# Natasha-R/Flood-Prediction-GAN

Measured on AMD Instinct MI355X. Metric: GAN training images/sec (512x512, PairedAttention), higher is better.
Workload: dtype f32

## Files before the change

### flood-prediction-gan_amd/csrc/conv_common.hpp

```cpp
#pragma once
#include "fg_common.hpp"

typedef _Float16 f16x8 __attribute__((ext_vector_type(8)));
typedef _Float16 f16x4 __attribute__((ext_vector_type(4)));
typedef _Float16 f16x2 __attribute__((ext_vector_type(2)));
typedef float f32x2 __attribute__((ext_vector_type(2)));

namespace fgc {

struct ConvBatch {
    fg_conv_problem p[4];
    int count;
    int ntiles_n[4];
    int blk_start[5];
    int interleave;
};

__device__ __forceinline__ int div_small(int n, int d) {
    int q = (int)((float)n * __builtin_amdgcn_rcpf((float)d));
    const int r = n - q * d;
    q += r >= d ? 1 : (r < 0 ? -1 : 0);
    return q;
}

// ... 13 lines not shown

__device__ __forceinline__ float pow2_of(float m) {
    if (!(m > 0.f) || !(m < 3.0e38f)) return 1.f;
    int e;
    frexpf(m, &e);
    return ldexpf(1.f, 14 - e);
}

__device__ __forceinline__ float pow2_scale_max(const float* amax) {
    unsigned b = __float_as_uint(amax[threadIdx.x & (FG_AMAX_SHARDS - 1)]) & 0x7fffffffu;
#pragma unroll
    for (int off = 1; off < FG_AMAX_SHARDS; off <<= 1) b = max(b, (unsigned)__shfl_xor((int)b, off));
    return __uint_as_float(b);
}

__device__ __forceinline__ float pow2_scale(const float* amax) {
    unsigned b = amax ? __float_as_uint(amax[threadIdx.x & (FG_AMAX_SHARDS - 1)]) & 0x7fffffffu : 0u;
#pragma unroll
    for (int off = 1; off < FG_AMAX_SHARDS; off <<= 1) b = max(b, (unsigned)__shfl_xor((int)b, off));
    return pow2_of(__uint_as_float(b));
}

__device__ __forceinline__ void split_f16(const float (&v)[8], float s, f16x8& h, f16x8& l) {
#pragma unroll
    for (int e = 0; e < 4; ++e) {
        const f32x2 x = f32x2{v[2 * e], v[2 * e + 1]} * s;
        const f16x2 hh = __builtin_convertvector(x, f16x2);
        const f16x2 ll = __builtin_convertvector(x - __builtin_convertvector(hh, f32x2), f16x2);
        h[2 * e] = hh[0];
        h[2 * e + 1] = hh[1];
        l[2 * e] = ll[0];
        l[2 * e + 1] = ll[1];
    }
}

__device__ __forceinline__ void split_pair_mix(float x0, float x1, float s, unsigned& h, unsigned& l) {
    unsigned hv, lv;
    asm("v_fma_mixlo_f16 %0, %1, %2, 0\n\t"
        "v_fma_mixhi_f16 %0, %3, %2, 0"
        : "=&v"(hv) : "v"(x0), "v"(s), "v"(x1));
    asm("v_fma_mixlo_f16 %0, %1, %2, -%4 op_sel_hi:[0,0,1]\n\t"
        "v_fma_mixhi_f16 %0, %3, %2, -%4 op_sel:[0,0,1] op_sel_hi:[0,0,1]"
        : "=&v"(lv) : "v"(x0), "v"(s), "v"(x1), "v"(hv));
    h = hv;
    l = lv;
}

template <int C>
__device__ __forceinline__ int swz_pixel(int x) {
    if constexpr (C == 64) return (x & 7) << 1;
    else return ((x >> 1) & 3) << 1;
}

int launch_fwd_f3(const ConvBatch& b, int nprob, int max_n, hipStream_t stream, int* rc);
bool f3_stats_ok(const fg_conv_problem* probs, int nprob, int max_n);

int launch_wgrad_f3(const fg_wgrad_problem& p, hipStream_t stream, int* rc);

int stem_wgrad_rows(const fg_wgrad_problem& p);
int launch_wgrad_stem(const fg_wgrad_problem& p, hipStream_t stream, int* rc);
int stem_fwd_rows(const fg_conv_problem& p);
int launch_fwd_stem(const fg_conv_problem& p, hipStream_t stream, int* rc);

}
```

### flood-prediction-gan_amd/csrc/conv_f3.hip

```cpp
#include <algorithm>

#include "conv_common.hpp"

namespace {

using fgc::ConvBatch;

__device__ __forceinline__ int swz_a(int row) { return ((row >> 1) & 1) ^ (((row >> 3) & 1) << 2); }
__device__ __forceinline__ int swz_b(int row) { return ((row >> 3) & 1) << 1; }

typedef __attribute__((address_space(3))) void lds_void;
typedef unsigned u32x4 __attribute__((ext_vector_type(4)));

__device__ __forceinline__ void split_scalar(const float (&v)[8], float s, f16x8& h, f16x8& l) {
#pragma unroll
    for (int e = 0; e < 4; ++e) {
        const float x0 = v[2 * e] * s, x1 = v[2 * e + 1] * s;
        const f16x2 hh = __builtin_convertvector(f32x2{x0, x1}, f16x2);
        const float r0 = x0 - (float)hh[0], r1 = x1 - (float)hh[1];
        const f16x2 ll = __builtin_convertvector(f32x2{r0, r1}, f16x2);
        h[2 * e] = hh[0];
        h[2 * e + 1] = hh[1];
        l[2 * e] = ll[0];
        l[2 * e + 1] = ll[1];
    }
}

template <int A_GL, int B_GL, int A_BYTES>
__device__ __forceinline__ void dma_stage(char* sb, int wave, __amdgpu_buffer_rsrc_t xr, __amdgpu_buffer_rsrc_t wr,
                                          const int* a_off, const int* b_off, int soff_a, int soff_b) {
#pragma unroll
    for (int i = 0; i < A_GL; ++i)
        __builtin_amdgcn_raw_ptr_buffer_load_lds(xr, (lds_void*)(sb + (wave * A_GL + i) * 1024), 16, a_off[i], soff_a,
                                                 0, 0);
#pragma unroll
    for (int i = 0; i < B_GL; ++i)
        __builtin_amdgcn_raw_ptr_buffer_load_lds(wr, (lds_void*)(sb + A_BYTES + (wave * B_GL + i) * 1024), 16, b_off[i],
                                                 soff_b, 0, 0);
}

__device__ __forceinline__ f32x4 mma_t(f16x8 a, f16x8 b, f32x4 c) {
    return __builtin_amdgcn_mfma_f32_16x16x32_f16(b, a, c, 0, 0, 0);
}

__device__ __forceinline__ int quad_yoff(const fg_conv_problem& P, int q) {
    const int y0 = (int)P.q_yoff[0], y1 = (int)P.q_yoff[1], y2 = (int)P.q_yoff[2], y3 = (int)P.q_yoff[3];
    return q == 0 ? y0 : q == 1 ? y1 : q == 2 ? y2 : y3;
}

constexpr int kYRecords = 0x7fffff00, kYOOB = 0x7ffffff0;

__device__ __forceinline__ void dma_piece(char* dst, __amdgpu_buffer_rsrc_t r, int voff, int soff) {
    __builtin_amdgcn_raw_ptr_buffer_load_lds(r, (lds_void*)dst, 16, voff, soff, 0, 0);
}

constexpr int cap63(int n) { return n < 63 ? n : 63; }

template <int N>
__device__ __forceinline__ void wait_vmcnt() {
    static_assert(N >= 0 && N <= 63, "vmcnt immediate (6 bits)");
    asm volatile("s_waitcnt vmcnt(%0)" ::"n"(N) : "memory");
}

__device__ __forceinline__ void wait_vmcnt_rt(int n) {
    switch (n < 63 ? n : 63) {
        case 0: wait_vmcnt<0>(); break;
        case 1: wait_vmcnt<1>(); break;
        case 2: wait_vmcnt<2>(); break;
        case 3: wait_vmcnt<3>(); break;
        case 4: wait_vmcnt<4>(); break;
        case 5: wait_vmcnt<5>(); break;
        case 6: wait_vmcnt<6>(); break;
        case 7: wait_vmcnt<7>(); break;
        case 8: wait_vmcnt<8>(); break;
        case 9: wait_vmcnt<9>(); break;
        case 10: wait_vmcnt<10>(); break;
        case 11: wait_vmcnt<11>(); break;
        case 12: wait_vmcnt<12>(); break;
        case 13: wait_vmcnt<13>(); break;
        case 14: wait_vmcnt<14>(); break;
        case 15: wait_vmcnt<15>(); break;
        case 16: wait_vmcnt<16>(); break;
        case 17: wait_vmcnt<17>(); break;
        case 18: wait_vmcnt<18>(); break;
        case 19: wait_vmcnt<19>(); break;
        case 20: wait_vmcnt<20>(); break;
        case 21: wait_vmcnt<21>(); break;
        case 22: wait_vmcnt<22>(); break;
        case 23: wait_vmcnt<23>(); break;
        case 24: wait_vmcnt<24>(); break;
        case 25: wait_vmcnt<25>(); break;
        case 26: wait_vmcnt<26>(); break;
        case 27: wait_vmcnt<27>(); break;
        case 28: wait_vmcnt<28>(); break;
        case 29: wait_vmcnt<29>(); break;
        case 30: wait_vmcnt<30>(); break;
        case 31: wait_vmcnt<31>(); break;
        case 32: wait_vmcnt<32>(); break;
        case 33: wait_vmcnt<33>(); break;
        case 34: wait_vmcnt<34>(); break;
        case 35: wait_vmcnt<35>(); break;
        case 36: wait_vmcnt<36>(); break;
        case 37: wait_vmcnt<37>(); break;
        case 38: wait_vmcnt<38>(); break;
        case 39: wait_vmcnt<39>(); break;
        case 40: wait_vmcnt<40>(); break;
        case 41: wait_vmcnt<41>(); break;
        case 42: wait_vmcnt<42>(); break;
        case 43: wait_vmcnt<43>(); break;
        case 44: wait_vmcnt<44>(); break;
        case 45: wait_vmcnt<45>(); break;
        case 46: wait_vmcnt<46>(); break;
        case 47: wait_vmcnt<47>(); break;
        case 48: wait_vmcnt<48>(); break;
        case 49: wait_vmcnt<49>(); break;
// ... 785 lines not shown
```

### flood-prediction-gan_amd/csrc/conv_wgrad_f3.hip

```cpp
#include "conv_common.hpp"

namespace {

typedef short s16x4 __attribute__((ext_vector_type(4)));
typedef __attribute__((address_space(3))) s16x4 lds_s16x4;

constexpr int BR = 32;
constexpr int TK = 256;

__device__ __forceinline__ int swz_tr(int row) { return ((row & 3) | (((row >> 3) & 1) << 2)) << 1; }

template <int COLS>
__device__ __forceinline__ int img_off(int row, int col) {
    return row * (COLS * 2) + (((col >> 3) ^ (swz_tr(row) & (COLS / 8 - 1))) << 4) + ((col & 7) << 1);
}

__device__ __forceinline__ f16x8 tr_frag(const char* base, int a0, int a1) {
    const s16x4 lo = __builtin_amdgcn_ds_read_tr16_b64_v4i16((lds_s16x4*)(base + a0));
    const s16x4 hi = __builtin_amdgcn_ds_read_tr16_b64_v4i16((lds_s16x4*)(base + a1));
    typedef short s16x8 __attribute__((ext_vector_type(8)));
    const s16x8 v = {lo[0], lo[1], lo[2], lo[3], hi[0], hi[1], hi[2], hi[3]};
    return __builtin_bit_cast(f16x8, v);
}

__device__ __forceinline__ void split4(const f32x4& v, float s, f16x4& h, f16x4& l) {
    typedef unsigned u32x2 __attribute__((ext_vector_type(2)));
    u32x2 hu, lu;
#pragma unroll
    for (int e = 0; e < 2; ++e) {
        unsigned a, b;
        fgc::split_pair_mix(v[2 * e], v[2 * e + 1], s, a, b);
        hu[e] = a;
        lu[e] = b;
    }
    h = __builtin_bit_cast(f16x4, hu);
    l = __builtin_bit_cast(f16x4, lu);
}

template <int TA, int SCH, int PS = 0>
__global__ void __launch_bounds__(512, 1)
conv_wgrad_f3_kernel(const fg_wgrad_problem P, int tiles_a, int tiles_k) {
    constexpr int NT = 512, NWA = TA / 64, NWK = 8 / NWA, WK = TK / NWK, TM = 4, TN = WK / 16;
    constexpr int SPT = BR * TK / 4 / NT;
    constexpr int IMGP = BR * TA * 2, IMGX = BR * TK * 2;
    constexpr int PL = IMGP + 64, XH = 2 * IMGP + 128, XL = XH + IMGX + 64;
    constexpr int BUF = XL + IMGX + 64;
    constexpr int kOOB = 0x7fffffff;
    __shared__ __attribute__((aligned(1024))) char smem[2 * BUF];

    const int tid = threadIdx.x, lane = tid & 63, wave = __builtin_amdgcn_readfirstlane(tid >> 6);
    const int wa = wave / NWK, wk = wave - (wave / NWK) * NWK;
    const int wid = fg::xcd_remap(blockIdx.x, gridDim.x);
    const int ntile = tiles_a * tiles_k;
    const int split = wid / ntile;
    const int tile = wid - split * ntile;
    const int ta = tile / tiles_k, tk = tile - (tile / tiles_k) * tiles_k;
    const int a0 = ta * TA, k0 = tk * TK;
    const int mab = P.m_a * P.m_b;
    const int M = P.m_img * mab;
    const int mbeg = split * P.m_chunk;
    const int mend = min(M, mbeg + P.m_chunk);
    const int K = P.kh * P.j_valid;
    const int nst = mend > mbeg ? (mend - mbeg + BR - 1) / BR : 0;

    const __amdgpu_buffer_rsrc_t pr = __builtin_amdgcn_make_buffer_rsrc((void*)P.p, 0, 0x7fffffff, 0x00020000);
    const __amdgpu_buffer_rsrc_t xr = __builtin_amdgcn_make_buffer_rsrc((void*)P.x, 0, 0x7fffffff, 0x00020000);
    const float sp = fgc::pow2_scale(P.p_absmax);
    const float sx = fgc::pow2_scale(P.x_absmax);

    const int col = (tid & 63) * 4;
    const int prow0 = wave;
    const bool p_slot = col < TA;
    const bool p_col_ok = p_slot && a0 + col < P.n_a;
    int x_koff = -1;
    {
        const int k = k0 + col;
        if (k < K) {
            const int r = k / P.j_valid;
            x_koff = r * (int)P.sxr + (k - r * P.j_valid);
        }
    }
    const int i32 = BR / mab, a32 = (BR - i32 * mab) / P.m_b, b32 = BR - i32 * mab - a32 * P.m_b;
    int wm[SPT], wi[SPT], wa_[SPT], wb[SPT];
#pragma unroll
    for (int i = 0; i < SPT; ++i) {
        wm[i] = mbeg + prow0 + 8 * i;
        fgc::decomp(min(wm[i], M - 1), P.m_b, mab, wi[i], wa_[i], wb[i]);
    }
    f32x4 rp[SPT], rx[SPT];
    auto load_slot = [&](int i) {
        {
            const bool ok = wm[i] < mend;
            const int pb = wi[i] * (int)P.spn + wa_[i] * (int)P.spa + wb[i] * (int)P.spb + a0 + col;
            const int xb = wi[i] * (int)P.sxn + wa_[i] * (int)P.sxa + wb[i] * (int)P.sxb + x_koff;
            rp[i] = __builtin_bit_cast(f32x4, __builtin_amdgcn_raw_buffer_load_b128(pr, ok && p_col_ok ? pb * 4 : kOOB, 0, 0));
            rx[i] = __builtin_bit_cast(f32x4, __builtin_amdgcn_raw_buffer_load_b128(xr, ok && x_koff >= 0 ? xb * 4 : kOOB, 0, 0));
            wm[i] += BR;
            wb[i] += b32;
            const int cb = wb[i] >= P.m_b;
            wb[i] -= cb ? P.m_b : 0;
            wa_[i] += a32 + cb;
            const int ca = wa_[i] >= P.m_a;
            wa_[i] -= ca ? P.m_a : 0;
            wi[i] += i32 + ca;
        }
    };
    auto load = [&]() {
#pragma unroll
        for (int i = 0; i < SPT; ++i) load_slot(i);
    };
    auto store_slot = [&](int buf, int i) {
        char* b = smem + buf * BUF;
        {
            f16x4 h, l;
            if (p_slot) {
                if constexpr (PS & 1) {
                    const int op = img_off<TA>(prow0 + 8 * i, col & ~7) + ((col & 4) ? PL : 0);
                    *reinterpret_cast<f16x8*>(b + op) = __builtin_bit_cast(f16x8, rp[i]);
                } else {
                    const int op = img_off<TA>(prow0 + 8 * i, col);
                    split4(rp[i], sp, h, l);
                    *reinterpret_cast<f16x4*>(b + op) = h;
                    *reinterpret_cast<f16x4*>(b + PL + op) = l;
                }
            }
            if constexpr (PS & 2) {
                const int ox = img_off<TK>(prow0 + 8 * i, col & ~7) + ((col & 4) ? XL : XH);
                *reinterpret_cast<f16x8*>(b + ox) = __builtin_bit_cast(f16x8, rx[i]);
            } else {
                const int ox = img_off<TK>(prow0 + 8 * i, col);
                split4(rx[i], sx, h, l);
                *reinterpret_cast<f16x4*>(b + XH + ox) = h;
                *reinterpret_cast<f16x4*>(b + XL + ox) = l;
            }
        }
    };
    auto store = [&](int buf) {
#pragma unroll
        for (int i = 0; i < SPT; ++i) store_slot(buf, i);
    };

    f32x4 acc[TM][TN];
#pragma unroll
    for (int tm = 0; tm < TM; ++tm)
#pragma unroll
        for (int tn = 0; tn < TN; ++tn) acc[tm][tn] = f32x4{0.f, 0.f, 0.f, 0.f};

    const int g = lane >> 4, q = (lane >> 2) & 3, p4 = (lane & 3) * 4;
    constexpr int TG = SCH == 0 ? (TN < 4 ? TN : 4) : TN / SPT;
    static_assert(TN % TG == 0 && (SCH == 0 || TN / TG == SPT), "groups");
    auto compute = [&](int buf, bool stage_next) {
        const char* b = smem + buf * BUF;
        f16x8 ah[TM], al[TM];
#pragma unroll
        for (int tm = 0; tm < TM; ++tm) {
            const int c = wa * 64 + tm * 16 + p4;
            const int o0 = img_off<TA>(8 * g + q, c), o1 = img_off<TA>(8 * g + 4 + q, c);
            ah[tm] = tr_frag(b, o0, o1);
            al[tm] = tr_frag(b + PL, o0, o1);
        }
#pragma unroll
        for (int t0 = 0; t0 < TN; t0 += TG) {
            f16x8 bh[TG], bl[TG];
#pragma unroll
            for (int t = 0; t < TG; ++t) {
                const int c = wk * WK + (t0 + t) * 16 + p4;
                const int o0 = img_off<TK>(8 * g + q, c), o1 = img_off<TK>(8 * g + 4 + q, c);
                bh[t] = tr_frag(b + XH, o0, o1);
                bl[t] = tr_frag(b + XL, o0, o1);
            }
            if constexpr (SCH == 1) {
                if (stage_next) store_slot(buf ^ 1, t0 / TG);
                load_slot(t0 / TG);
            }
#pragma unroll
            for (int tm = 0; tm < TM; ++tm)
#pragma unroll
                for (int t = 0; t < TG; ++t)
                    acc[tm][t0 + t] = __builtin_amdgcn_mfma_f32_16x16x32_f16(bh[t], al[tm], acc[tm][t0 + t], 0, 0, 0);
#pragma unroll
            for (int tm = 0; tm < TM; ++tm)
#pragma unroll
                for (int t = 0; t < TG; ++t)
                    acc[tm][t0 + t] = __builtin_amdgcn_mfma_f32_16x16x32_f16(bl[t], ah[tm], acc[tm][t0 + t], 0, 0, 0);
#pragma unroll
            for (int tm = 0; tm < TM; ++tm)
#pragma unroll
                for (int t = 0; t < TG; ++t)
                    acc[tm][t0 + t] = __builtin_amdgcn_mfma_f32_16x16x32_f16(bh[t], ah[tm], acc[tm][t0 + t], 0, 0, 0);
        }
    };

    load();
    store(0);
    load();
    __syncthreads();
    for (int st = 0; st < nst; ++st) {
        const int cur = st & 1;
        if constexpr (SCH == 0) {
            if (st + 1 < nst) store(cur ^ 1);
            load();
            __builtin_amdgcn_sched_barrier(0);
            compute(cur, false);
        } else {
            compute(cur, st + 1 < nst);
        }
        __syncthreads();
    }

    float* out = P.out + (size_t)split * P.n_a * K;
    const float osc = 1.f / (sp * sx);
    const int fr = lane & 15;
#pragma unroll
    for (int tm = 0; tm < TM; ++tm) {
        const int a = a0 + wa * 64 + tm * 16 + fr;
        if (a >= P.n_a) continue;
#pragma unroll
        for (int tn = 0; tn < TN; ++tn) {
            const int k = k0 + wk * WK + tn * 16 + 4 * g;
            if (k < K) *reinterpret_cast<f32x4*>(out + (size_t)a * K + k) = acc[tm][tn] * osc;
        }
    }
}

}

int g_wgrad_f3 = 2;

namespace fgc {

int launch_wgrad_f3(const fg_wgrad_problem& p, hipStream_t stream, int* rc) {
    if (!g_wgrad_f3 || p.n_a < 64 || p.kh * p.j_valid < 256 || p.n_a % 4 || p.j_valid % 4 || !p.p_absmax ||
        !p.x_absmax || ((uintptr_t)p.p & 15) || ((uintptr_t)p.x & 15) || (p.spn | p.spa | p.spb) % 4 ||
        (p.sxn | p.sxa | p.sxb | p.sxr) % 4)
        return 0;
    const int TA = p.n_a >= 256 ? 256 : p.n_a > 64 ? 128 : 64;
    const int ta = (p.n_a + TA - 1) / TA, tk = (p.kh * p.j_valid + TK - 1) / TK;
    const dim3 grid(ta * tk * p.splits);
    const int ps = (p.p_presplit ? 1 : 0) | (p.x_presplit ? 2 : 0);
    if (ps) {
        if (p.n_a % 8 || p.j_valid % 8 || (p.p_presplit && (((uintptr_t)p.p & 31) || (p.spn | p.spa | p.spb) % 8)) ||
            (p.x_presplit && (((uintptr_t)p.x & 31) || (p.sxn | p.sxa | p.sxb | p.sxr) % 8)))
            return 0;
        if (TA == 64) {
            if (ps == 1)
                FG_LAUNCH((conv_wgrad_f3_kernel<64, 0, 1>), grid, dim3(512), 0, stream, p, ta, tk);
            else if (ps == 2)
                FG_LAUNCH((conv_wgrad_f3_kernel<64, 0, 2>), grid, dim3(512), 0, stream, p, ta, tk);
            else
                FG_LAUNCH((conv_wgrad_f3_kernel<64, 0, 3>), grid, dim3(512), 0, stream, p, ta, tk);
        } else if (TA == 256) {
            if (ps == 1)
                FG_LAUNCH((conv_wgrad_f3_kernel<256, 0, 1>), grid, dim3(512), 0, stream, p, ta, tk);
            else if (ps == 2)
                FG_LAUNCH((conv_wgrad_f3_kernel<256, 0, 2>), grid, dim3(512), 0, stream, p, ta, tk);
            else
                FG_LAUNCH((conv_wgrad_f3_kernel<256, 0, 3>), grid, dim3(512), 0, stream, p, ta, tk);
        } else {
            if (ps == 1)
                FG_LAUNCH((conv_wgrad_f3_kernel<128, 1, 1>), grid, dim3(512), 0, stream, p, ta, tk);
            else if (ps == 2)
                FG_LAUNCH((conv_wgrad_f3_kernel<128, 1, 2>), grid, dim3(512), 0, stream, p, ta, tk);
            else
                FG_LAUNCH((conv_wgrad_f3_kernel<128, 1, 3>), grid, dim3(512), 0, stream, p, ta, tk);
        }
        *rc = fg::launched("conv_wgrad_f3_presplit");
        return 1;
    }
    const int sch = g_wgrad_f3 == 3 || (g_wgrad_f3 == 2 && TA == 128) ? 1 : 0;
    if (TA == 64)
        FG_LAUNCH((conv_wgrad_f3_kernel<64, 0>), grid, dim3(512), 0, stream, p, ta, tk);
    else if (TA == 256 && sch == 1)
        FG_LAUNCH((conv_wgrad_f3_kernel<256, 1>), grid, dim3(512), 0, stream, p, ta, tk);
    else if (TA == 256)
        FG_LAUNCH((conv_wgrad_f3_kernel<256, 0>), grid, dim3(512), 0, stream, p, ta, tk);
    else if (sch == 1)
        FG_LAUNCH((conv_wgrad_f3_kernel<128, 1>), grid, dim3(512), 0, stream, p, ta, tk);
    else
        FG_LAUNCH((conv_wgrad_f3_kernel<128, 0>), grid, dim3(512), 0, stream, p, ta, tk);
    *rc = fg::launched("conv_wgrad_f3");
    return 1;
}

}

FG_API int fg_set_wgrad_f3(int on) {
    if (on < 0 || on > 3) return fg::fail(FG_ERR_INVALID, "fg_set_wgrad_f3: %d", on);
    g_wgrad_f3 = on;
    return 0;
}
```

### flood-prediction-gan_amd/floodgan/_lib.py

```python
import ctypes as C
import os

import torch

_HERE = os.path.dirname(os.path.abspath(__file__))
LIB_PATH = os.environ.get("FLOODGAN_LIB", os.path.join(_HERE, "lib", "libfloodgan.so"))

FG_PAD_ZERO, FG_PAD_REFLECT = 0, 1
FG_ACT_NONE, FG_ACT_RELU, FG_ACT_LRELU = 0, 1, 2
FG_MATH_FP32, FG_MATH_FWD_X6, FG_MATH_WGRAD_X6, FG_MATH_BF16X6 = 0, 1, 2, 3
FG_MATH_FWD_F16X3, FG_MATH_WGRAD_F16X3, FG_MATH_F16X3 = 4, 8, 12
CONV_MATH = {"fp32": FG_MATH_FP32, "fwd_x6": FG_MATH_FWD_X6, "wgrad_x6": FG_MATH_WGRAD_X6, "bf16x6": FG_MATH_BF16X6,
             "fwd_f16x3": FG_MATH_FWD_F16X3, "wgrad_f16x3": FG_MATH_WGRAD_F16X3, "f16x3": FG_MATH_F16X3}


class fg_view(C.Structure):
    _fields_ = [("ptr", C.c_void_p), ("n", C.c_int), ("h", C.c_int), ("w", C.c_int),
                ("c_alloc", C.c_int), ("pad", C.c_int)]


class fg_sview(C.Structure):
    _fields_ = [("ptr", C.c_void_p), ("sn", C.c_longlong), ("sc", C.c_longlong),
                ("sy", C.c_longlong), ("sx", C.c_longlong)]

# ... 38 lines not shown


class fg_adam_tensor(C.Structure):
    _fields_ = [("param", C.c_void_p), ("grad", C.c_void_p), ("exp_avg", C.c_void_p),
                ("exp_avg_sq", C.c_void_p), ("numel", C.c_longlong), ("absmax", C.c_void_p)]


FG_TILE_MAX_CH = 16

FG_RENDER_SIGNED, FG_RENDER_UNIT = 0, 1
FG_SCALAR_UNIT, FG_SCALAR_THRESHOLD, FG_SCALAR_LOGIT = 0, 1, 2


class fg_canvas(C.Structure):
    _fields_ = [("ptr", C.c_void_p), ("height", C.c_int), ("width", C.c_int), ("row_bytes", C.c_longlong)]

F3_ORDER_DEFAULT = 31


class fg_tile_batch(C.Structure):
    _fields_ = [("src", C.c_void_p), ("tile_stride", C.c_longlong),
                ("n", C.c_int), ("h_in", C.c_int), ("w_in", C.c_int), ("c_src", C.c_int),
                ("flip", C.c_void_p), ("c_out", C.c_int), ("chan", C.c_int * FG_TILE_MAX_CH),
                ("crop", C.c_void_p), ("row_lo", C.c_void_p), ("rows", C.c_int), ("out_h", C.c_int), ("out_w", C.c_int),
                ("x_idx0", C.c_void_p), ("x_w", C.c_void_p), ("x_taps", C.c_int),
                ("y_idx0", C.c_void_p), ("y_w", C.c_void_p), ("y_taps", C.c_int),
                ("tmp", C.c_void_p), ("dst", fg_wview)]


SIGNATURES = {
    "fg_last_error": [],
    "fg_last_launch": [],
    "fg_version": [],
    "fg_device_ok": [],
    "fg_timing_event_create": [C.c_int, C.POINTER(C.c_void_p)],
    "fg_timing_event_record": [C.c_void_p, C.c_void_p],
    "fg_timing_event_elapsed": [C.c_void_p, C.c_void_p, C.POINTER(C.c_float)],
    "fg_timing_event_destroy": [C.c_void_p],
    "fg_timing_arm": [C.c_void_p, C.c_void_p],
    "fg_timing_disarm": [],
    "fg_conv_fwd": [C.POINTER(fg_conv_problem), C.c_int, C.c_void_p],
    "fg_conv_stats_ok": [C.POINTER(fg_conv_problem), C.c_int],
    "fg_set_conv_math": [C.c_int],
    "fg_get_conv_math": [],
    "fg_set_fwd_tile": [C.c_int],
    "fg_set_wgrad_tile": [C.c_int],
    "fg_set_f3_tile": [C.c_int],
    "fg_set_f3_order": [C.c_int],
    "fg_set_f3_sched": [C.c_int],
    "fg_set_f3_persistent": [C.c_int],
    "fg_set_f3_fill": [C.c_int],
    "fg_set_f3_interleave": [C.c_int],
    "fg_set_wgrad_f3": [C.c_int],
    "fg_set_in_rows": [C.c_int],
    "fg_set_f3_ps_wide": [C.c_int],
    "fg_set_f3_ps_tall": [C.c_int],
    "fg_conv_wgrad": [C.POINTER(fg_wgrad_problem), C.c_void_p],
    "fg_wgrad_reduce": [C.c_void_p, C.c_int, C.POINTER(fg_weight_map), C.c_void_p, C.c_int, C.c_void_p],
    "fg_pack_weight": [C.c_void_p, C.POINTER(fg_weight_map), C.c_void_p, C.c_void_p],
    "fg_pack_weight_split": [C.c_void_p, C.POINTER(fg_weight_map), C.c_void_p, C.c_void_p],
    "fg_pack_weight_f16": [C.c_void_p, C.POINTER(fg_weight_map), C.c_void_p, C.c_void_p, C.c_void_p],
    "fg_pack_weight_f16_batch": [C.c_void_p, C.c_int, C.c_void_p],
    "fg_absmax": [C.c_void_p, C.c_longlong, C.c_void_p, C.c_void_p],
    "fg_conv_n1_fwd": [C.c_void_p, C.c_int, C.c_int, C.c_int, C.c_int, C.c_void_p, C.c_void_p, C.c_void_p, C.c_int,
                       C.c_int, C.c_void_p],
    "fg_conv_n1_wgrad_blocks": [C.c_int, C.c_int, C.c_int],
    "fg_conv_n1_wgrad": [C.c_void_p, C.c_int, C.c_int, C.c_int, C.c_int, C.c_void_p, C.c_int, C.c_int, C.c_int,
                         C.c_void_p, C.c_void_p],
    "fg_d0_input_grad": [fg_view, C.c_void_p, C.c_int, C.c_int, C.c_int, C.c_void_p, C.c_int, C.c_int, C.c_int,
                         C.c_int, C.c_void_p],
    "fg_split_pixels": [C.c_void_p, C.c_longlong, C.c_int, C.c_int, C.c_void_p, C.c_void_p, C.c_void_p],
    "fg_conv_win": [C.POINTER(fg_conv_problem), C.c_void_p, C.c_longlong, C.c_void_p],
    "fg_conv_wgrad_win": [C.POINTER(fg_wgrad_problem), C.c_void_p, C.c_longlong, C.c_int, C.c_int, C.c_void_p,
                          C.c_longlong, C.c_int, C.c_void_p],
    "fg_conv1x1_fwd": [fg_view, C.c_void_p, C.c_void_p, C.c_int, fg_view, C.c_void_p],
    "fg_conv1x1_dgrad": [fg_view, C.c_void_p, C.c_int, fg_view, C.c_void_p],
    "fg_conv1x1_wgrad": [fg_view, fg_view, C.c_int, C.c_void_p, C.c_void_p, C.c_int, C.c_void_p, C.c_void_p],
    "fg_conv1x1_wgrad_workspace_floats": [C.c_int],
    "fg_pack_input": [fg_sview, C.c_int, fg_sview, C.c_int, fg_view, C.c_int, C.c_int, C.c_int, C.c_void_p, C.c_void_p],
    "fg_zero_border": [fg_view, C.c_void_p],
    "fg_fold_add": [fg_view, C.c_int, fg_view, fg_view, C.c_void_p],
    "fg_unfold_nchw": [fg_view, C.c_int, C.c_int, fg_wview, C.c_int, C.c_int, C.c_int, C.c_void_p],
    "fg_in_workspace_doubles": [C.c_int, C.c_int],
    "fg_in_stats": [fg_view, C.c_float, C.c_void_p, C.c_void_p, C.c_void_p, C.c_void_p],
    "fg_in_stats_partials": [C.c_void_p, C.c_int, C.c_int, C.c_int, C.c_int, C.c_float, C.c_void_p, C.c_void_p,
                             C.c_void_p, C.c_void_p],
    "fg_in_partials_workspace_doubles": [C.c_int, C.c_int],
    "fg_in_apply": [fg_view, C.c_void_p, C.c_void_p, C.c_int, fg_view, fg_view, C.c_int, C.c_void_p, C.c_void_p],
    "fg_in_bwd": [fg_view, C.c_int, fg_view, fg_view, C.c_void_p, C.c_void_p, C.c_int, fg_view, C.c_void_p,
                  C.c_int, fg_view, C.c_void_p, C.c_void_p, C.c_void_p],
    "fg_in_apply_presplit": [fg_view, C.c_void_p, C.c_void_p, C.c_int, fg_view, C.c_int, C.c_void_p, C.c_void_p],
    "fg_in_apply_splitpix": [fg_view, C.c_void_p, C.c_void_p, C.c_int, fg_view, C.c_int, C.c_void_p, C.c_void_p],
    "fg_in_apply_dual": [fg_view, C.c_void_p, C.c_void_p, C.c_int, fg_view, C.c_void_p, fg_view, C.c_int, C.c_void_p,
                         C.c_void_p, C.c_void_p, C.c_void_p],
    "fg_in_apply_head": [fg_view, C.c_void_p, C.c_void_p, C.c_int, fg_view, C.c_int, C.c_void_p, C.c_void_p,
                         C.c_void_p, C.c_int, fg_view, C.c_void_p],
    "fg_in_bwd_head": [fg_view, C.c_void_p, C.c_int, fg_view, C.c_void_p, C.c_void_p, C.c_int, fg_view, C.c_void_p,
                       C.c_int, C.c_void_p, C.c_void_p, C.c_void_p, C.c_void_p, C.c_void_p, C.c_int, C.c_void_p,
                       C.c_void_p],
    "fg_in_head_wgrad_workspace_floats": [C.c_int, C.c_int, C.c_int, C.c_int],
    "fg_in_bwd_presplit": [fg_view, C.c_int, fg_view, fg_view, C.c_void_p, C.c_void_p, C.c_int, fg_view, C.c_void_p,
                           C.c_int, fg_view, C.c_void_p, C.c_void_p, C.c_void_p],
    "fg_act_bwd": [fg_view, fg_view, C.c_int, C.c_void_p, C.c_void_p],
    "fg_channel_sum": [fg_view, C.c_int, C.c_void_p, C.c_int, C.c_void_p, C.c_void_p],
    "fg_channel_sum_workspace_doubles": [C.c_int],
    "fg_tail_fwd": [fg_view, fg_view, fg_sview, C.c_void_p, C.c_void_p, C.c_void_p],
# ... 65 lines not shown
    for name, argt in SIGNATURES.items():
        fn = getattr(lib, name)
        fn.argtypes = argt
        fn.restype = RESTYPES.get(name, C.c_int)
    _lib = lib
    mode = os.environ.get("FLOODGAN_CONV_MATH")
    if mode:
        set_conv_math(mode)
    return lib


def set_conv_math(mode):
    check(load().fg_set_conv_math(CONV_MATH[mode]), "set_conv_math")


def fwd_x6():
    return bool(load().fg_get_conv_math() & FG_MATH_FWD_X6)


def fwd_f16x3():
    return bool(load().fg_get_conv_math() & FG_MATH_FWD_F16X3)


def wgrad_f16x3():
    return bool(load().fg_get_conv_math() & FG_MATH_WGRAD_F16X3)


def set_fwd_tile(cfg):
    check(load().fg_set_fwd_tile(int(cfg)), "set_fwd_tile")


def set_wgrad_tile(cfg):
    check(load().fg_set_wgrad_tile(int(cfg)), "set_wgrad_tile")


def set_f3_tile(cfg):
    check(load().fg_set_f3_tile(int(cfg)), "set_f3_tile")


_WGRAD_F3 = True


def set_wgrad_f3(mode):
    global _WGRAD_F3
    mode = 2 if mode is True else int(mode)
    check(load().fg_set_wgrad_f3(mode), "set_wgrad_f3")
    _WGRAD_F3 = mode != 0


def wgrad_f3_on():
    return _WGRAD_F3


def get_conv_math():
    inv = {v: k for k, v in CONV_MATH.items()}
    return inv[load().fg_get_conv_math()]


def check(rc, what):
    if rc != 0:
        msg = load().fg_last_error().decode(errors="replace")
        raise RuntimeError(f"floodgan {what} failed (code {rc}): {msg}")


def stream_handle(device=None):
    s = torch.cuda.current_stream(device)
    return C.c_void_p(s.cuda_stream)


def ptr(t):
    return C.c_void_p(t.data_ptr()) if t is not None else C.c_void_p(0)


def require_device(t, what="tensor"):
    if not (t.is_cuda and t.dtype == torch.float32):
        raise RuntimeError(f"floodgan: {what} must be a float32 tensor on a HIP device "
                           f"(got {t.dtype} on {t.device}); there is no CPU path")


def last_launch():
    return load().fg_last_launch().decode()
```

### include/floodgan.h

```cpp
#ifndef FLOODGAN_H
#define FLOODGAN_H

#include <hip/hip_runtime.h>

#ifdef __cplusplus
extern "C" {
#endif


enum { FG_PAD_ZERO = 0, FG_PAD_REFLECT = 1 };
enum { FG_ACT_NONE = 0, FG_ACT_RELU = 1, FG_ACT_LRELU = 2 };
enum { FG_ERR_INVALID = -1 };
enum { FG_AMAX_SHARDS = 64 };
enum {
    FG_MATH_FP32 = 0,
    FG_MATH_FWD_X6 = 1,
    FG_MATH_WGRAD_X6 = 2,
    FG_MATH_BF16X6 = 3,
    FG_MATH_FWD_F16X3 = 4,
    FG_MATH_WGRAD_F16X3 = 8,
    FG_MATH_F16X3 = 12
};

typedef struct fg_view {
// ... 42 lines not shown
    long long spn, spa, spb;
    long long sxn, sxa, sxb, sxr;
    int m_img, m_a, m_b;
    int n_a, kh, j_valid;
    int splits, m_chunk;
    const float* p_absmax;
    const float* x_absmax;
    int p_presplit, x_presplit;
} fg_wgrad_problem;

typedef struct fg_weight_map {
    int n_out;
    int kh, kw, c;
    int c_valid;
    int jp;
    int dim0_is_n;
    int d0, d1, KH, KW;
    int n_base;
    int rtab[8];
    int stab[8];
    int q_n;
} fg_weight_map;

const char* fg_last_error(void);
const char* fg_last_launch(void);
int fg_version(void);
int fg_device_ok(void);
int fg_timing_event_create(int mode, void** ev);
int fg_timing_event_record(void* ev, hipStream_t stream);
int fg_timing_event_elapsed(void* start, void* end, float* ms);
int fg_timing_event_destroy(void* ev);
int fg_timing_arm(void* start, void* stop);
int fg_timing_disarm(void);

int fg_conv_fwd(const fg_conv_problem* probs, int nprob, hipStream_t stream);

int fg_conv_stats_ok(const fg_conv_problem* probs, int nprob);

int fg_set_conv_math(int mode);
int fg_get_conv_math(void);

int fg_set_fwd_tile(int cfg);
int fg_set_wgrad_tile(int cfg);
int fg_set_f3_tile(int cfg);
int fg_set_f3_order(int alt);
int fg_set_f3_sched(int sched);
int fg_set_f3_persistent(int on);
int fg_set_f3_fill(int on);
int fg_set_f3_ps_wide(int cfg);
int fg_set_f3_ps_tall(int on);
int fg_set_f3_interleave(int on);
int fg_set_in_rows(int on);
int fg_set_wgrad_f3(int on);

int fg_conv_wgrad(const fg_wgrad_problem* prob, hipStream_t stream);

int fg_wgrad_reduce(const float* slabs, int splits, const fg_weight_map* map, float* dw,
                    int accumulate, hipStream_t stream);

int fg_pack_weight(const float* w, const fg_weight_map* map, float* wp, hipStream_t stream);

int fg_pack_weight_split(const float* w, const fg_weight_map* map, void* wps, hipStream_t stream);

int fg_pack_weight_f16(const float* w, const fg_weight_map* map, const float* w_absmax, void* wps,
                       hipStream_t stream);

typedef struct fg_pack_job {
    const float* w;
    const float* w_absmax;
    void* dst;
    fg_weight_map map;
} fg_pack_job;

#define FG_PACK_BATCH_MAX 24
int fg_pack_weight_f16_batch(const fg_pack_job* jobs, int njobs, hipStream_t stream);

int fg_split_pixels(const float* src, long long npix, int c, int wp, const float* amax, void* dst,
                    hipStream_t stream);

int fg_conv_win(const fg_conv_problem* prob, const void* x_split, long long x_pix0, hipStream_t stream);

int fg_conv_wgrad_win(const fg_wgrad_problem* prob, const void* p_split, long long p_pix0, int p_col0,
                      int wp_p, const void* x_split, long long x_pix0, int wp_x, hipStream_t stream);

int fg_conv1x1_fwd(fg_view x, const float* w, const float* bias, int n_out, fg_view y, hipStream_t stream);
int fg_conv1x1_dgrad(fg_view gy, const float* w, int n_out, fg_view gx, hipStream_t stream);
long long fg_conv1x1_wgrad_workspace_floats(int n_out);
int fg_conv1x1_wgrad(fg_view gy, fg_view x, int n_out, float* dw, float* db, int accumulate, float* work,
                     hipStream_t stream);

int fg_conv_n1_fwd(const float* x, int nimg, int hp, int wp, int c, const float* w, const float* bias,
                   float* y, int ho, int wo, hipStream_t stream);
int fg_conv_n1_wgrad_blocks(int nimg, int hp, int rows_per_block);
int fg_conv_n1_wgrad(const float* x, int nimg, int hp, int wp, int c, const float* gp, int ghp, int gwp,
                     int rows_per_block, float* slabs, hipStream_t stream);

int fg_d0_input_grad(fg_view g, const float* w, int ctot, int c0, int cn, float* y, int yc, int H, int W,
                     int accumulate, hipStream_t stream);

int fg_absmax(const float* x, long long n, float* out, hipStream_t stream);

int fg_pack_input(fg_sview a, int ca, fg_sview b, int cb, fg_view dst, int img0, int nimg,
                  int pad_mode, float* absmax, hipStream_t stream);

int fg_zero_border(fg_view dst, hipStream_t stream);

// ... 157 lines not shown
```

Measured before the change: 177.5.

## Stage pre-split wgrad operands into LDS via buffer-load-to-LDS DMA

Adds a DMA path to the f16x3 weight-gradient kernel for pre-split operands. Global loads now write straight into a swizzled LDS image with buffer_load ... lds, skipping the register round-trip and the ds_write stores, and the next stage is issued at the start of compute. Compile-time checks verify that the swizzle is free of bank conflicts. It is on by default for the 256-wide tile only, and it adds inline-asm m0 handling and a full vmcnt(0) wait every stage, which may limit overlap.

```diff
diff --git a/flood-prediction-gan_amd/csrc/conv_common.hpp b/flood-prediction-gan_amd/csrc/conv_common.hpp
--- a/flood-prediction-gan_amd/csrc/conv_common.hpp
+++ b/flood-prediction-gan_amd/csrc/conv_common.hpp
@@ -89,6 +89,18 @@
     else return ((x >> 1) & 3) << 1;
 }
 
+typedef __attribute__((address_space(3))) void lds_void;
+
+__device__ __forceinline__ void dma_piece(char* dst, __amdgpu_buffer_rsrc_t r, int voff, int soff) {
+    __builtin_amdgcn_raw_ptr_buffer_load_lds(r, (lds_void*)dst, 16, voff, soff, 0, 0);
+}
+
+template <int N>
+__device__ __forceinline__ void wait_vmcnt() {
+    static_assert(N >= 0 && N <= 63, "vmcnt immediate (6 bits)");
+    asm volatile("s_waitcnt vmcnt(%0)" ::"n"(N) : "memory");
+}
+
 int launch_fwd_f3(const ConvBatch& b, int nprob, int max_n, hipStream_t stream, int* rc);
 bool f3_stats_ok(const fg_conv_problem* probs, int nprob, int max_n);
 
diff --git a/flood-prediction-gan_amd/csrc/conv_f3.hip b/flood-prediction-gan_amd/csrc/conv_f3.hip
--- a/flood-prediction-gan_amd/csrc/conv_f3.hip
+++ b/flood-prediction-gan_amd/csrc/conv_f3.hip
@@ -9,7 +9,7 @@
 __device__ __forceinline__ int swz_a(int row) { return ((row >> 1) & 1) ^ (((row >> 3) & 1) << 2); }
 __device__ __forceinline__ int swz_b(int row) { return ((row >> 3) & 1) << 1; }
 
-typedef __attribute__((address_space(3))) void lds_void;
+using fgc::lds_void;
 typedef unsigned u32x4 __attribute__((ext_vector_type(4)));
 
 __device__ __forceinline__ void split_scalar(const float (&v)[8], float s, f16x8& h, f16x8& l) {
@@ -50,17 +50,10 @@
 
 constexpr int kYRecords = 0x7fffff00, kYOOB = 0x7ffffff0;
 
-__device__ __forceinline__ void dma_piece(char* dst, __amdgpu_buffer_rsrc_t r, int voff, int soff) {
-    __builtin_amdgcn_raw_ptr_buffer_load_lds(r, (lds_void*)dst, 16, voff, soff, 0, 0);
-}
+using fgc::dma_piece;
+using fgc::wait_vmcnt;
 
 constexpr int cap63(int n) { return n < 63 ? n : 63; }
-
-template <int N>
-__device__ __forceinline__ void wait_vmcnt() {
-    static_assert(N >= 0 && N <= 63, "vmcnt immediate (6 bits)");
-    asm volatile("s_waitcnt vmcnt(%0)" ::"n"(N) : "memory");
-}
 
 __device__ __forceinline__ void wait_vmcnt_rt(int n) {
     switch (n < 63 ? n : 63) {
diff --git a/flood-prediction-gan_amd/csrc/conv_wgrad_f3.hip b/flood-prediction-gan_amd/csrc/conv_wgrad_f3.hip
--- a/flood-prediction-gan_amd/csrc/conv_wgrad_f3.hip
+++ b/flood-prediction-gan_amd/csrc/conv_wgrad_f3.hip
@@ -13,6 +13,62 @@
 template <int COLS>
 __device__ __forceinline__ int img_off(int row, int col) {
     return row * (COLS * 2) + (((col >> 3) ^ (swz_tr(row) & (COLS / 8 - 1))) << 4) + ((col & 7) << 1);
+}
+
+constexpr int dma_swz(int row) { return (row & 1) | (((row >> 1) & 1) << 2) | (((row >> 3) & 1) << 3); }
+template <int COLS>
+constexpr int dma_row(int row) { return COLS == 256 ? row : (row & 7) * 4 + (row >> 3); }
+template <int COLS>
+constexpr int dma_off(int row, int col, int piece) {
+    return dma_row<COLS>(row) * (COLS * 4) + (((2 * (col >> 3) + piece) ^ dma_swz(row)) << 4) + ((col & 7) << 1);
+}
+template <int COLS>
+constexpr bool dma_img_ok() {
+    for (int rd = 0; rd < 2; ++rd)
+        for (int hf = 0; hf < 2; ++hf)
+            for (int c0 = 0; c0 < COLS; c0 += 16)
+                for (int pc = 0; pc < 2; ++pc) {
+                    unsigned long long used = 0;
+                    for (int l = 0; l < 32; ++l) {
+                        const int g = 2 * hf + (l >> 4), q = (l >> 2) & 3, p4 = (l & 3) * 4;
+                        const int a = dma_off<COLS>(8 * g + 4 * rd + q, c0 + p4, pc);
+                        if (a & 7) return false;
+                        for (int d = 0; d < 2; ++d) {
+                            const unsigned long long bit = 1ull << ((a / 4 + d) % 64);
+                            if (used & bit) return false;
+                            used |= bit;
+                        }
+                    }
+                }
+    for (int row = 0; row < BR; ++row)
+        for (int cb = 0; cb < COLS; cb += 64)
+            for (int t = 0; t < (cb % 128 ? 4 : 8) && cb + 16 * t < COLS; ++t)
+                for (int pc = 0; pc < 2; ++pc)
+                    for (int p4 = 0; p4 < 16; p4 += 4) {
+                        if (dma_off<COLS>(row, cb + 16 * t + p4, pc) != (dma_off<COLS>(row, cb + p4, 0) ^ ((4 * t + pc) << 4)))
+                            return false;
+                        if ((row & 4) == 0 && dma_off<COLS>(row + 4, cb + p4, 0) - dma_off<COLS>(row, cb + p4, 0) !=
+                                                  dma_off<COLS>(4, 0, 0))
+                            return false;
+                    }
+    return true;
+}
+static_assert(dma_img_ok<256>(), "LDS-DMA image, 1-KB rows (X, and P of the 256-row tile): bank conflict or address form");
+static_assert(dma_img_ok<128>(), "LDS-DMA image, 512-B rows (P of the 128-row tile): bank conflict or address form");
+
+typedef unsigned u32x4 __attribute__((ext_vector_type(4)));
+__device__ __forceinline__ void dma_piece_uncounted(unsigned lds, u32x4 rsrc, int voff, int soff) {
+    unsigned keep;
+    asm volatile("s_mov_b32 %0, m0\n\t"
+                 "s_mov_b32 m0, %1\n\t"
+                 "s_nop 4\n\t"
+                 "buffer_load_dwordx4 %2, %3, %4 offen lds\n\t"
+                 "s_mov_b32 m0, %0"
+                 : "=&s"(keep) : "s"(lds), "v"(voff), "s"(rsrc), "s"(soff) : "memory");
+}
+__device__ __forceinline__ u32x4 raw_rsrc(const void* p) {
+    const unsigned long long a = (unsigned long long)p;
+    return u32x4{(unsigned)a, (unsigned)(a >> 32) & 0xffffu, 0x7fffffffu, 0x00020000u};
 }
 
 __device__ __forceinline__ f16x8 tr_frag(const char* base, int a0, int a1) {
@@ -37,7 +93,7 @@
     l = __builtin_bit_cast(f16x4, lu);
 }
 
-template <int TA, int SCH, int PS = 0>
+template <int TA, int SCH, int PS = 0, int DMA = 0>
 __global__ void __launch_bounds__(512, 1)
 conv_wgrad_f3_kernel(const fg_wgrad_problem P, int tiles_a, int tiles_k) {
     constexpr int NT = 512, NWA = TA / 64, NWK = 8 / NWA, WK = TK / NWK, TM = 4, TN = WK / 16;
@@ -45,8 +101,10 @@
     constexpr int IMGP = BR * TA * 2, IMGX = BR * TK * 2;
     constexpr int PL = IMGP + 64, XH = 2 * IMGP + 128, XL = XH + IMGX + 64;
     constexpr int BUF = XL + IMGX + 64;
+    constexpr int DBUF = 2 * (IMGP + IMGX);
     constexpr int kOOB = 0x7fffffff;
-    __shared__ __attribute__((aligned(1024))) char smem[2 * BUF];
+    static_assert(!DMA || (PS == 3 && SCH == 0 && (TA == 256 || TA == 128)), "LDS-DMA staging: pre-split operands");
+    __shared__ __attribute__((aligned(1024))) char smem[2 * (DMA ? DBUF : BUF)];
 
     const int tid = threadIdx.x, lane = tid & 63, wave = __builtin_amdgcn_readfirstlane(tid >> 6);
     const int wa = wave / NWK, wk = wave - (wave / NWK) * NWK;
@@ -68,18 +126,7 @@
     const float sp = fgc::pow2_scale(P.p_absmax);
     const float sx = fgc::pow2_scale(P.x_absmax);
 
-    const int col = (tid & 63) * 4;
     const int prow0 = wave;
-    const bool p_slot = col < TA;
-    const bool p_col_ok = p_slot && a0 + col < P.n_a;
-    int x_koff = -1;
-    {
-        const int k = k0 + col;
-        if (k < K) {
-            const int r = k / P.j_valid;
-            x_koff = r * (int)P.sxr + (k - r * P.j_valid);
-        }
-    }
     const int i32 = BR / mab, a32 = (BR - i32 * mab) / P.m_b, b32 = BR - i32 * mab - a32 * P.m_b;
     int wm[SPT], wi[SPT], wa_[SPT], wb[SPT];
 #pragma unroll
@@ -87,125 +134,244 @@
         wm[i] = mbeg + prow0 + 8 * i;
         fgc::decomp(min(wm[i], M - 1), P.m_b, mab, wi[i], wa_[i], wb[i]);
     }
-    f32x4 rp[SPT], rx[SPT];
-    auto load_slot = [&](int i) {
+    auto advance_slot = [&](int i) {
+        wm[i] += BR;
+        wb[i] += b32;
+        const int cb = wb[i] >= P.m_b;
+        wb[i] -= cb ? P.m_b : 0;
+        wa_[i] += a32 + cb;
+        const int ca = wa_[i] >= P.m_a;
+        wa_[i] -= ca ? P.m_a : 0;
+        wi[i] += i32 + ca;
+    };
+
+    f32x4 acc[TM][TN];
+#pragma unroll
+    for (int tm = 0; tm < TM; ++tm)
+#pragma unroll
+        for (int tn = 0; tn < TN; ++tn) acc[tm][tn] = f32x4{0.f, 0.f, 0.f, 0.f};
+
+    const int g = lane >> 4, q = (lane >> 2) & 3, p4 = (lane & 3) * 4;
+
+    if constexpr (DMA) {
+        constexpr int IP = 2 * IMGP;
+        int xv[2], pv[2];
+#pragma unroll
+        for (int par = 0; par < 2; ++par) {
+            const int sw = dma_swz(prow0 + 8 * par);
+            int k = k0 + 4 * (lane ^ sw);
+            k = k < K ? k : k0;
+            const int r = k / P.j_valid;
+            xv[par] = (r * (int)P.sxr + (k - r * P.j_valid)) * 4;
+            const int a = a0 + 4 * ((TA == 256 ? lane : lane & 31) ^ sw);
+            pv[par] = (a < P.n_a ? a : a0) * 4;
+        }
+        int p_safe;
         {
-            const bool ok = wm[i] < mend;
-            const int pb = wi[i] * (int)P.spn + wa_[i] * (int)P.spa + wb[i] * (int)P.spb + a0 + col;
-            const int xb = wi[i] * (int)P.sxn + wa_[i] * (int)P.sxa + wb[i] * (int)P.sxb + x_koff;
-            rp[i] = __builtin_bit_cast(f32x4, __builtin_amdgcn_raw_buffer_load_b128(pr, ok && p_col_ok ? pb * 4 : kOOB, 0, 0));
-            rx[i] = __builtin_bit_cast(f32x4, __builtin_amdgcn_raw_buffer_load_b128(xr, ok && x_koff >= 0 ? xb * 4 : kOOB, 0, 0));
-            wm[i] += BR;
-            wb[i] += b32;
-            const int cb = wb[i] >= P.m_b;
-            wb[i] -= cb ? P.m_b : 0;
-            wa_[i] += a32 + cb;
-            const int ca = wa_[i] >= P.m_a;
-            wa_[i] -= ca ? P.m_a : 0;
-            wi[i] += i32 + ca;
-        }
-    };
-    auto load = [&]() {
-#pragma unroll
-        for (int i = 0; i < SPT; ++i) load_slot(i);
-    };
-    auto store_slot = [&](int buf, int i) {
-        char* b = smem + buf * BUF;
+            int si, sa, sb;
+            fgc::decomp(min(mbeg, M - 1), P.m_b, mab, si, sa, sb);
+            p_safe = si * (int)P.spn + sa * (int)P.spa + sb * (int)P.spb;
+        }
+        int pws[SPT];
+        const u32x4 pd = raw_rsrc(P.p), xd = raw_rsrc(P.x);
+        const unsigned lds0 = (unsigned)(size_t)(__attribute__((address_space(3))) char*)smem;
+        auto issue_slot = [&](int buf, int i, bool ragged) {
+            const bool ok = !ragged || wm[i] < mend;
+            const int xs = wi[i] * (int)P.sxn + wa_[i] * (int)P.sxa + wb[i] * (int)P.sxb;
+            const int ps = ok ? wi[i] * (int)P.spn + wa_[i] * (int)P.spa + wb[i] * (int)P.spb : p_safe;
+            const int d = __builtin_amdgcn_readfirstlane(buf * DBUF + (prow0 + 8 * i) * 1024);
+            if (ok)
+                dma_piece_uncounted(lds0 + d + IP, xd, xv[i & 1], xs * 4);
+            else
+                *reinterpret_cast<f32x4*>(smem + d + IP + lane * 16) = f32x4{0.f, 0.f, 0.f, 0.f};
+            if constexpr (TA == 256) {
+                dma_piece_uncounted(lds0 + d, pd, pv[i & 1], ps * 4);
+            } else {
+                pws[i] = ps;
+                if (i & 1) {
+                    const int dp = __builtin_amdgcn_readfirstlane(buf * DBUF + (prow0 * 2 + (i >> 1)) * 1024);
+                    dma_piece_uncounted(lds0 + dp, pd, ((lane & 32) ? pws[i] : pws[i - 1]) * 4 + pv[(lane >> 5) & 1], 0);
+                }
+            }
+            advance_slot(i);
+        };
+
+        const int abase = dma_off<TA>(8 * g + q, wa * 64 + p4, 0), xbase = IP + dma_off<TK>(8 * g + q, wk * WK + p4, 0);
+        constexpr int A4 = dma_off<TA>(4, 0, 0), X4 = dma_off<TK>(4, 0, 0);
+        constexpr int TG = TN < 4 ? TN : 4;
+        static_assert(TN % TG == 0, "groups");
+        auto compute = [&](int buf, int stage_next) {
+            const char* b = smem + buf * DBUF;
+            f16x8 ah[TM], al[TM];
+            if (stage_next == 1) {
+#pragma unroll
+                for (int i = 0; i < SPT; ++i) issue_slot(buf ^ 1, i, false);
+            } else if (stage_next == 2) {
+#pragma unroll
+                for (int i = 0; i < SPT; ++i) issue_slot(buf ^ 1, i, true);
+            }
+#pragma unroll
+            for (int tm = 0; tm < TM; ++tm) {
+                const int oh = abase ^ ((4 * tm) << 4), ol = abase ^ ((4 * tm + 1) << 4);
+                ah[tm] = tr_frag(b, oh, oh + A4);
+                al[tm] = tr_frag(b, ol, ol + A4);
+            }
+#pragma unroll
+            for (int t0 = 0; t0 < TN; t0 += TG) {
+                f16x8 bh[TG], bl[TG];
+#pragma unroll
+                for (int t = 0; t < TG; ++t) {
+                    const int oh = xbase ^ ((4 * (t0 + t)) << 4), ol = xbase ^ ((4 * (t0 + t) + 1) << 4);
+                    bh[t] = tr_frag(b, oh, oh + X4);
+                    bl[t] = tr_frag(b, ol, ol + X4);
+                }
+#pragma unroll
+                for (int tm = 0; tm < TM; ++tm)
+#pragma unroll
+                    for (int t = 0; t < TG; ++t)
+                        acc[tm][t0 + t] = __builtin_amdgcn_mfma_f32_16x16x32_f16(bh[t], al[tm], acc[tm][t0 + t], 0, 0, 0);
+#pragma unroll
+                for (int tm = 0; tm < TM; ++tm)
+#pragma unroll
+                    for (int t = 0; t < TG; ++t)
+                        acc[tm][t0 + t] = __builtin_amdgcn_mfma_f32_16x16x32_f16(bl[t], ah[tm], acc[tm][t0 + t], 0, 0, 0);
+#pragma unroll
+                for (int tm = 0; tm < TM; ++tm)
+#pragma unroll
+                    for (int t = 0; t < TG; ++t)
+                        acc[tm][t0 + t] = __builtin_amdgcn_mfma_f32_16x16x32_f16(bh[t], ah[tm], acc[tm][t0 + t], 0, 0, 0);
+            }
+        };
+
+        if (nst > 0) {
+#pragma unroll
+            for (int i = 0; i < SPT; ++i) issue_slot(0, i, true);
+        }
+        fgc::wait_vmcnt<0>();
+        __syncthreads();
+        for (int st = 0; st < nst; ++st) {
+            compute(st & 1, st + 1 >= nst ? 0 : mbeg + (st + 2) * BR <= mend ? 1 : 2);
+            fgc::wait_vmcnt<0>();
+            __syncthreads();
+        }
+    } else {
+        const int col = (tid & 63) * 4;
+        const bool p_slot = col < TA;
+        const bool p_col_ok = p_slot && a0 + col < P.n_a;
+        int x_koff = -1;
         {
-            f16x4 h, l;
-            if (p_slot) {
-                if constexpr (PS & 1) {
-                    const int op = img_off<TA>(prow0 + 8 * i, col & ~7) + ((col & 4) ? PL : 0);
-                    *reinterpret_cast<f16x8*>(b + op) = __builtin_bit_cast(f16x8, rp[i]);
+            const int k = k0 + col;
+            if (k < K) {
+                const int r = k / P.j_valid;
+                x_koff = r * (int)P.sxr + (k - r * P.j_valid);
+            }
+        }
+        f32x4 rp[SPT], rx[SPT];
+        auto load_slot = [&](int i) {
+            {
+                const bool ok = wm[i] < mend;
+                const int pb = wi[i] * (int)P.spn + wa_[i] * (int)P.spa + wb[i] * (int)P.spb + a0 + col;
+                const int xb = wi[i] * (int)P.sxn + wa_[i] * (int)P.sxa + wb[i] * (int)P.sxb + x_koff;
+                rp[i] = __builtin_bit_cast(f32x4, __builtin_amdgcn_raw_buffer_load_b128(pr, ok && p_col_ok ? pb * 4 : kOOB, 0, 0));
+                rx[i] = __builtin_bit_cast(f32x4, __builtin_amdgcn_raw_buffer_load_b128(xr, ok && x_koff >= 0 ? xb * 4 : kOOB, 0, 0));
+                advance_slot(i);
+            }
+        };
+        auto load = [&]() {
+#pragma unroll
+            for (int i = 0; i < SPT; ++i) load_slot(i);
+        };
+        auto store_slot = [&](int buf, int i) {
+            char* b = smem + buf * BUF;
+            {
+                f16x4 h, l;
+                if (p_slot) {
+                    if constexpr (PS & 1) {
+                        const int op = img_off<TA>(prow0 + 8 * i, col & ~7) + ((col & 4) ? PL : 0);
+                        *reinterpret_cast<f16x8*>(b + op) = __builtin_bit_cast(f16x8, rp[i]);
+                    } else {
+                        const int op = img_off<TA>(prow0 + 8 * i, col);
+                        split4(rp[i], sp, h, l);
+                        *reinterpret_cast<f16x4*>(b + op) = h;
+                        *reinterpret_cast<f16x4*>(b + PL + op) = l;
+                    }
+                }
+                if constexpr (PS & 2) {
+                    const int ox = img_off<TK>(prow0 + 8 * i, col & ~7) + ((col & 4) ? XL : XH);
+                    *reinterpret_cast<f16x8*>(b + ox) = __builtin_bit_cast(f16x8, rx[i]);
                 } else {
-                    const int op = img_off<TA>(prow0 + 8 * i, col);
-                    split4(rp[i], sp, h, l);
-                    *reinterpret_cast<f16x4*>(b + op) = h;
-                    *reinterpret_cast<f16x4*>(b + PL + op) = l;
-                }
-            }
-            if constexpr (PS & 2) {
-                const int ox = img_off<TK>(prow0 + 8 * i, col & ~7) + ((col & 4) ? XL : XH);
-                *reinterpret_cast<f16x8*>(b + ox) = __builtin_bit_cast(f16x8, rx[i]);
+                    const int ox = img_off<TK>(prow0 + 8 * i, col);
+                    split4(rx[i], sx, h, l);
+                    *reinterpret_cast<f16x4*>(b + XH + ox) = h;
+                    *reinterpret_cast<f16x4*>(b + XL + ox) = l;
+                }
+            }
+        };
+        auto store = [&](int buf) {
+#pragma unroll
+            for (int i = 0; i < SPT; ++i) store_slot(buf, i);
+        };
+
+        constexpr int TG = SCH == 0 ? (TN < 4 ? TN : 4) : TN / SPT;
+        static_assert(TN % TG == 0 && (SCH == 0 || TN / TG == SPT), "groups");
+        auto compute = [&](int buf, bool stage_next) {
+            const char* b = smem + buf * BUF;
+            f16x8 ah[TM], al[TM];
+#pragma unroll
+            for (int tm = 0; tm < TM; ++tm) {
+                const int c = wa * 64 + tm * 16 + p4;
+                const int o0 = img_off<TA>(8 * g + q, c), o1 = img_off<TA>(8 * g + 4 + q, c);
+                ah[tm] = tr_frag(b, o0, o1);
+                al[tm] = tr_frag(b + PL, o0, o1);
+            }
+#pragma unroll
+            for (int t0 = 0; t0 < TN; t0 += TG) {
+                f16x8 bh[TG], bl[TG];
+#pragma unroll
+                for (int t = 0; t < TG; ++t) {
+                    const int c = wk * WK + (t0 + t) * 16 + p4;
+                    const int o0 = img_off<TK>(8 * g + q, c), o1 = img_off<TK>(8 * g + 4 + q, c);
+                    bh[t] = tr_frag(b + XH, o0, o1);
+                    bl[t] = tr_frag(b + XL, o0, o1);
+                }
+                if constexpr (SCH == 1) {
+                    if (stage_next) store_slot(buf ^ 1, t0 / TG);
+                    load_slot(t0 / TG);
+                }
+#pragma unroll
+                for (int tm = 0; tm < TM; ++tm)
+#pragma unroll
+                    for (int t = 0; t < TG; ++t)
+                        acc[tm][t0 + t] = __builtin_amdgcn_mfma_f32_16x16x32_f16(bh[t], al[tm], acc[tm][t0 + t], 0, 0, 0);
+#pragma unroll
+                for (int tm = 0; tm < TM; ++tm)
+#pragma unroll
+                    for (int t = 0; t < TG; ++t)
+                        acc[tm][t0 + t] = __builtin_amdgcn_mfma_f32_16x16x32_f16(bl[t], ah[tm], acc[tm][t0 + t], 0, 0, 0);
+#pragma unroll
+                for (int tm = 0; tm < TM; ++tm)
+#pragma unroll
+                    for (int t = 0; t < TG; ++t)
+                        acc[tm][t0 + t] = __builtin_amdgcn_mfma_f32_16x16x32_f16(bh[t], ah[tm], acc[tm][t0 + t], 0, 0, 0);
+            }
+        };
+
+        load();
+        store(0);
+        load();
+        __syncthreads();
+        for (int st = 0; st < nst; ++st) {
+            const int cur = st & 1;
+            if constexpr (SCH == 0) {
+                if (st + 1 < nst) store(cur ^ 1);
+                load();
+                __builtin_amdgcn_sched_barrier(0);
+                compute(cur, false);
             } else {
-                const int ox = img_off<TK>(prow0 + 8 * i, col);
-                split4(rx[i], sx, h, l);
-                *reinterpret_cast<f16x4*>(b + XH + ox) = h;
-                *reinterpret_cast<f16x4*>(b + XL + ox) = l;
-            }
-        }
-    };
-    auto store = [&](int buf) {
-#pragma unroll
-        for (int i = 0; i < SPT; ++i) store_slot(buf, i);
-    };
-
-    f32x4 acc[TM][TN];
-#pragma unroll
-    for (int tm = 0; tm < TM; ++tm)
-#pragma unroll
-        for (int tn = 0; tn < TN; ++tn) acc[tm][tn] = f32x4{0.f, 0.f, 0.f, 0.f};
-
-    const int g = lane >> 4, q = (lane >> 2) & 3, p4 = (lane & 3) * 4;
-    constexpr int TG = SCH == 0 ? (TN < 4 ? TN : 4) : TN / SPT;
-    static_assert(TN % TG == 0 && (SCH == 0 || TN / TG == SPT), "groups");
-    auto compute = [&](int buf, bool stage_next) {
-        const char* b = smem + buf * BUF;
-        f16x8 ah[TM], al[TM];
-#pragma unroll
-        for (int tm = 0; tm < TM; ++tm) {
-            const int c = wa * 64 + tm * 16 + p4;
-            const int o0 = img_off<TA>(8 * g + q, c), o1 = img_off<TA>(8 * g + 4 + q, c);
-            ah[tm] = tr_frag(b, o0, o1);
-            al[tm] = tr_frag(b + PL, o0, o1);
-        }
-#pragma unroll
-        for (int t0 = 0; t0 < TN; t0 += TG) {
-            f16x8 bh[TG], bl[TG];
-#pragma unroll
-            for (int t = 0; t < TG; ++t) {
-                const int c = wk * WK + (t0 + t) * 16 + p4;
-                const int o0 = img_off<TK>(8 * g + q, c), o1 = img_off<TK>(8 * g + 4 + q, c);
-                bh[t] = tr_frag(b + XH, o0, o1);
-                bl[t] = tr_frag(b + XL, o0, o1);
-            }
-            if constexpr (SCH == 1) {
-                if (stage_next) store_slot(buf ^ 1, t0 / TG);
-                load_slot(t0 / TG);
-            }
-#pragma unroll
-            for (int tm = 0; tm < TM; ++tm)
-#pragma unroll
-                for (int t = 0; t < TG; ++t)
-                    acc[tm][t0 + t] = __builtin_amdgcn_mfma_f32_16x16x32_f16(bh[t], al[tm], acc[tm][t0 + t], 0, 0, 0);
-#pragma unroll
-            for (int tm = 0; tm < TM; ++tm)
-#pragma unroll
-                for (int t = 0; t < TG; ++t)
-                    acc[tm][t0 + t] = __builtin_amdgcn_mfma_f32_16x16x32_f16(bl[t], ah[tm], acc[tm][t0 + t], 0, 0, 0);
-#pragma unroll
-            for (int tm = 0; tm < TM; ++tm)
-#pragma unroll
-                for (int t = 0; t < TG; ++t)
-                    acc[tm][t0 + t] = __builtin_amdgcn_mfma_f32_16x16x32_f16(bh[t], ah[tm], acc[tm][t0 + t], 0, 0, 0);
-        }
-    };
-
-    load();
-    store(0);
-    load();
-    __syncthreads();
-    for (int st = 0; st < nst; ++st) {
-        const int cur = st & 1;
-        if constexpr (SCH == 0) {
-            if (st + 1 < nst) store(cur ^ 1);
-            load();
-            __builtin_amdgcn_sched_barrier(0);
-            compute(cur, false);
-        } else {
-            compute(cur, st + 1 < nst);
-        }
-        __syncthreads();
+                compute(cur, st + 1 < nst);
+            }
+            __syncthreads();
+        }
     }
 
     float* out = P.out + (size_t)split * P.n_a * K;
@@ -223,9 +389,12 @@
     }
 }
 
+constexpr bool kDma256 = true, kDma128 = false;
+
 }
 
 int g_wgrad_f3 = 2;
+int g_wgrad_dma = 1;
 
 namespace fgc {
 
@@ -254,6 +423,8 @@
                 FG_LAUNCH((conv_wgrad_f3_kernel<256, 0, 1>), grid, dim3(512), 0, stream, p, ta, tk);
             else if (ps == 2)
                 FG_LAUNCH((conv_wgrad_f3_kernel<256, 0, 2>), grid, dim3(512), 0, stream, p, ta, tk);
+            else if (g_wgrad_dma == 2 || (g_wgrad_dma == 1 && kDma256))
+                FG_LAUNCH((conv_wgrad_f3_kernel<256, 0, 3, 1>), grid, dim3(512), 0, stream, p, ta, tk);
             else
                 FG_LAUNCH((conv_wgrad_f3_kernel<256, 0, 3>), grid, dim3(512), 0, stream, p, ta, tk);
         } else {
@@ -261,6 +432,8 @@
                 FG_LAUNCH((conv_wgrad_f3_kernel<128, 1, 1>), grid, dim3(512), 0, stream, p, ta, tk);
             else if (ps == 2)
                 FG_LAUNCH((conv_wgrad_f3_kernel<128, 1, 2>), grid, dim3(512), 0, stream, p, ta, tk);
+            else if (g_wgrad_dma == 2 || (g_wgrad_dma == 1 && kDma128))
+                FG_LAUNCH((conv_wgrad_f3_kernel<128, 0, 3, 1>), grid, dim3(512), 0, stream, p, ta, tk);
             else
                 FG_LAUNCH((conv_wgrad_f3_kernel<128, 1, 3>), grid, dim3(512), 0, stream, p, ta, tk);
         }
@@ -289,3 +462,9 @@
     g_wgrad_f3 = on;
     return 0;
 }
+
+FG_API int fg_set_wgrad_dma(int on) {
+    if (on < 0 || on > 2) return fg::fail(FG_ERR_INVALID, "fg_set_wgrad_dma: %d", on);
+    g_wgrad_dma = on;
+    return 0;
+}
diff --git a/flood-prediction-gan_amd/floodgan/_lib.py b/flood-prediction-gan_amd/floodgan/_lib.py
--- a/flood-prediction-gan_amd/floodgan/_lib.py
+++ b/flood-prediction-gan_amd/floodgan/_lib.py
@@ -114,6 +114,7 @@
     "fg_set_f3_fill": [C.c_int],
     "fg_set_f3_interleave": [C.c_int],
     "fg_set_wgrad_f3": [C.c_int],
+    "fg_set_wgrad_dma": [C.c_int],
     "fg_set_in_rows": [C.c_int],
     "fg_set_f3_ps_wide": [C.c_int],
     "fg_set_f3_ps_tall": [C.c_int],
@@ -285,6 +286,10 @@
     return _WGRAD_F3
 
 
+def set_wgrad_dma(on):
+    check(load().fg_set_wgrad_dma(int(on)), "set_wgrad_dma")
+
+
 def get_conv_math():
     inv = {v: k for k, v in CONV_MATH.items()}
     return inv[load().fg_get_conv_math()]
diff --git a/include/floodgan.h b/include/floodgan.h
--- a/include/floodgan.h
+++ b/include/floodgan.h
@@ -118,6 +118,7 @@
 int fg_set_f3_interleave(int on);
 int fg_set_in_rows(int on);
 int fg_set_wgrad_f3(int on);
+int fg_set_wgrad_dma(int on);
 
 int fg_conv_wgrad(const fg_wgrad_problem* prob, hipStream_t stream);
 
```

After: 178.9, median of 6. About the same (+0.8%).
